# qiaozhijian/LPD-Net-Pytorch

Measured on NVIDIA B200. Metric: LPD-Net eval embedding throughput (featnet=lpdnet, 4096 pts, k=20, NetVLAD K=64 D=1024 -> 256), higher is better.
Workload: dtype f16

## Files before the change

### include/lpd_b200.h

```cpp
#ifndef LPD_B200_H
#define LPD_B200_H

#include <stddef.h>
#include <stdint.h>

#ifdef __cplusplus
extern "C" {
#endif

#define LPD_ABI_VERSION 2

typedef enum lpd_status {
    LPD_OK = 0,
    LPD_EINVAL = -1,
    LPD_EWORKSPACE = -2,
    LPD_ECUDA = -3,
    LPD_EUNSUPPORTED = -4
} lpd_status;

typedef enum lpd_act {
    LPD_ACT_NONE = 0,
    LPD_ACT_RELU = 1,
    LPD_ACT_LEAKY = 2,
    LPD_ACT_SIGMOID = 3,
// ... 3 lines not shown

#define LPD_A_MK 0
#define LPD_A_KM 1
#define LPD_B_NK 0
#define LPD_B_KN 1

int lpd_abi_version(void);
const char* lpd_status_str(int status);
const char* lpd_last_cuda_error(void);
int lpd_device_info(int* sm_count, int* cc_major, int* cc_minor, size_t* smem_optin_bytes);

int lpd_bn_fold(const float* gamma, const float* beta, const float* mean, const float* var,
                const float* bias, float eps, int C, float* scale, float* shift, void* stream);

int lpd_transpose(const float* in, float* out, int batch, int rows, int cols, void* stream);

int lpd_knn(const float* x, int B, int N, int C, int k, void* idx, int idx_i64, void* stream);

size_t lpd_knn_workspace_bytes(int B, int N, int C, int k);
int lpd_knn_tc(const float* x, int B, int N, int C, int k, void* idx, int idx_i64,
               void* workspace, size_t workspace_bytes, void* stream);
int lpd_knn_tc_variant(int v);
size_t lpd_knn_tc_flags_offset(int B, int N, int C, int k);

size_t lpd_knn_xyz_workspace_bytes(int B, int N);
int lpd_knn_xyz(const float* x, int B, int N, int k, void* idx, int idx_i64, void* workspace, size_t workspace_bytes,
                void* stream);

int lpd_cell_order(const float* x, int B, int N, int32_t* perm, int32_t* inv, float* xyz_sorted,
                   void* workspace, size_t workspace_bytes, void* stream);

int lpd_cell_order_grid(const float* x, int B, int N, int32_t* perm, int32_t* inv, float* xyz_sorted,
                        void* workspace, size_t workspace_bytes, void* stream);
int lpd_knn_xyz_ordered(int B, int N, int k, void* idx, int idx_i64, void* workspace, size_t workspace_bytes, void* stream);

int lpd_gemm(const float* A, int a_layout, int lda, long long strideA,
             const float* B, int b_layout, int ldb, long long strideB,
             float* C, int ldc, long long strideC,
             int M, int N, int K, int batch,
             const float* scale, const float* shift, int act, float slope, const float* aux,
             void* stream);

int lpd_gemm_tf32(const float* A, int lda, const float* B, int ldb, float* C, int ldc,
                  int M, int N, int K, const float* scale, const float* shift, int act, float slope,
                  void* stream);
int lpd_gemm_tf32_ex(const float* A, int lda, const float* B, int ldb, float* C, int ldc,
// ... 140 lines not shown
```

### lpd-net-pytorch_b200/_lib.py

```python
from __future__ import annotations

import ctypes as C
import os
from pathlib import Path

_HERE = Path(__file__).resolve().parent
LIB_PATH = _HERE / "liblpd_b200.so"

LPD_OK = 0
ACT_NONE, ACT_RELU, ACT_LEAKY, ACT_SIGMOID, ACT_GATE, ACT_ADD = 0, 1, 2, 3, 4, 5
A_MK, A_KM = 0, 1
B_NK, B_KN = 0, 1
ABI_VERSION = 2

_vp, _i, _f, _ll, _sz, _d = C.c_void_p, C.c_int, C.c_float, C.c_longlong, C.c_size_t, C.c_double

SIGNATURES = {
    "lpd_abi_version": (_i, []),
    "lpd_status_str": (C.c_char_p, [_i]),
    "lpd_last_cuda_error": (C.c_char_p, []),
    "lpd_device_info": (_i, [C.POINTER(_i), C.POINTER(_i), C.POINTER(_i), C.POINTER(_sz)]),
    "lpd_bn_fold": (_i, [_vp, _vp, _vp, _vp, _vp, _f, _i, _vp, _vp, _vp]),
    "lpd_transpose": (_i, [_vp, _vp, _i, _i, _i, _vp]),
    "lpd_knn": (_i, [_vp, _i, _i, _i, _i, _vp, _i, _vp]),
    "lpd_knn_workspace_bytes": (_sz, [_i, _i, _i, _i]),
    "lpd_knn_tc": (_i, [_vp, _i, _i, _i, _i, _vp, _i, _vp, _sz, _vp]),
    "lpd_knn_tc_variant": (_i, [_i]),
    "lpd_knn_tc_flags_offset": (_sz, [_i, _i, _i, _i]),
    "lpd_knn_xyz_workspace_bytes": (_sz, [_i, _i]),
    "lpd_knn_xyz": (_i, [_vp, _i, _i, _i, _vp, _i, _vp, _sz, _vp]),
    "lpd_cell_order": (_i, [_vp, _i, _i, _vp, _vp, _vp, _vp, _sz, _vp]),
    "lpd_cell_order_grid": (_i, [_vp, _i, _i, _vp, _vp, _vp, _vp, _sz, _vp]),
    "lpd_knn_xyz_ordered": (_i, [_i, _i, _i, _vp, _i, _vp, _sz, _vp]),
    "lpd_gemm": (_i, [_vp, _i, _i, _ll, _vp, _i, _i, _ll, _vp, _i, _ll, _i, _i, _i, _i,
                      _vp, _vp, _i, _f, _vp, _vp]),
    "lpd_gemm_tf32": (_i, [_vp, _i, _vp, _i, _vp, _i, _i, _i, _i, _vp, _vp, _i, _f, _vp]),
    "lpd_gemm_tf32_ex": (_i, [_vp, _i, _vp, _i, _vp, _i, _i, _i, _i, _i, _i, _vp, _vp, _i, _f, _vp]),
    "lpd_gemm_tf32_tn": (_i, [_vp, _i, _vp, _i, _vp, _i, _ll, _i, _i, _i, _i, _vp]),
    "lpd_gemm_f16": (_i, [_vp, _i, _vp, _i, _vp, _i, _i, _i, _i, _i, _vp, _vp, _i, _f, _vp]),
    "lpd_gemm_f16_tn": (_i, [_vp, _i, _vp, _i, _vp, _i, _ll, _i, _i, _i, _i, _vp]),
    "lpd_f32_to_f16": (_i, [_vp, _ll, _vp, _ll, _ll, _i, _vp]),
    "lpd_split3_tf32": (_i, [_vp, _ll, _vp, _i, _vp]),
    "lpd_transpose_split3": (_i, [_vp, _i, _ll, _i, _vp, _vp]),
    "lpd_gemm_tf32_out16": (_i, [_vp, _i, _vp, _i, _vp, _i, _i, _i, _i, _vp, _vp, _i, _f, _vp]),
    "lpd_softmax64_f16": (_i, [_vp, _ll, _vp, _vp]),
    "lpd_edge_gather_max_f16": (_i, [_vp, _i, _vp, _i, _vp, _i, _i, _i, _i, _i, _f, _vp, _i, _vp]),
    "lpd_edgeconv_dg20_f16": (_i, [_vp, _i, _vp, _i, _vp, _i, _i, _vp, _vp, _vp, _i, _f, _vp, _i, _vp, _i, _vp]),
    "lpd_edgeconv_dg32_f16": (_i, [_vp, _i, _vp, _i, _vp, _i, _i, _vp, _vp, _vp, _i, _f, _vp, _i, _vp, _i, _vp]),
    "lpd_pointwise_mlp2": (_i, [_vp, _i, _i, _ll, _vp, _vp, _vp, _vp, _vp, _vp, _i, _f, _vp, _i, _vp]),
    "lpd_colmax": (_i, [_vp, _i, _i, _i, _i, _vp, _vp]),
    "lpd_edge_gather_ext": (_i, [_vp, _i, _vp, _i, _vp, _i, _i, _i, _i, _vp, _vp, _i, _f, _vp, _i, _vp]),
# ... 82 lines not shown
```

### lpd-net-pytorch_b200/csrc/knn_tc.cu

```cuda
#include "tc_common.cuh"
#include "knn_select.cuh"

namespace lpd {

int knn_simt64_flagged(const float* x, int B, int N, int k, void* idx, int idx_i64, const int* flags, cudaStream_t st);

namespace tc {

constexpr int KT_Q = 128;
constexpr int KT_C = 64;
constexpr int KT_SCAN_WARPS = 8;
constexpr int KT_THREADS = 320;
constexpr int KT_STRIDE = 257;
constexpr int KT_BSTAGES = 3;
constexpr int KT_TSTAGES = 4;
constexpr int KT_XSLOTS = 8;

struct KnnTcParams {
    const float* xxpad;
    float* cand_v;
    int* cand_i;
    int B, N, Npad;
    int qtiles, ctiles;
};
// ... 335 lines not shown
struct KnnWs {
    size_t off_xx, off_r2, off_flags, off_x2, off_cv, off_ci, total;
    int npad, L;
    KnnWs(int B, int N, int k) {
        npad = (N + 127) / 128 * 128;
        L = k <= 24 ? 48 : 64;
        size_t o = 0;
        off_xx = o; o = align_up(o + (size_t)B * npad * 4, 256);
        off_r2 = o; o += (size_t)B * 4;
        off_flags = o; o = align_up(o + (size_t)B * ((N + 63) / 64) * 4, 256);
        off_x2 = o; o = align_up(o + (size_t)B * N * 128 * 4, 256);
        off_cv = o; o = align_up(o + (size_t)B * N * L * 4, 256);
        off_ci = o; o = align_up(o + (size_t)B * N * L * 4, 256);
        total = o;
    }
};

}
}

namespace lpd { namespace tc {
size_t knn2_workspace_bytes(int B, int N, int k);
size_t knn2_flags_offset(int B, int N, int k);
int knn2_run(const float* x, int B, int N, int k, void* idx, int idx_i64, void* workspace, size_t workspace_bytes, int mt,
             cudaStream_t st);
static int g_knn_variant = 1;
}}

extern "C" int lpd_knn_tc_variant(int v) {
    const int prev = lpd::tc::g_knn_variant;
    if (v >= 0 && v <= 3) lpd::tc::g_knn_variant = v;
    return prev;
}

extern "C" size_t lpd_knn_workspace_bytes(int B, int N, int C, int k) {
    if (B < 1 || N < 1 || C != 64 || k < 1 || k > 32) return 0;
    const size_t a = lpd::tc::KnnWs(B, N, k).total, b = lpd::tc::knn2_workspace_bytes(B, N, k);
    return a > b ? a : b;
}

extern "C" size_t lpd_knn_tc_flags_offset(int B, int N, int C, int k) {
    if (B < 1 || N < 1 || C != 64 || k < 1 || k > 32) return 0;
    return lpd::tc::g_knn_variant == 0 ? lpd::tc::KnnWs(B, N, k).off_flags : lpd::tc::knn2_flags_offset(B, N, k);
}

extern "C" int lpd_knn_tc(const float* x, int B, int N, int C, int k, void* idx, int idx_i64,
                          void* workspace, size_t workspace_bytes, void* stream) {
    using namespace lpd;
    LPD_REQUIRE(x && idx && workspace);
    LPD_REQUIRE(B >= 1 && B <= 65535 && N >= 1 && C == 64 && k >= 1 && k <= 32 && k <= N);
    LPD_REQUIRE((long long)B * N < (1ll << 31) / 128);
    LPD_REQUIRE(((uintptr_t)x & 15) == 0 && ((uintptr_t)workspace & 255) == 0);
    const tc::KnnWs W(B, N, k);
    if (workspace_bytes < lpd_knn_workspace_bytes(B, N, C, k)) return LPD_EWORKSPACE;
    int dev = 0, major = 0;
    LPD_CUDA_CHECK(cudaGetDevice(&dev));
    LPD_CUDA_CHECK(cudaDeviceGetAttribute(&major, cudaDevAttrComputeCapabilityMajor, dev));
    if (major != 10) return LPD_EUNSUPPORTED;
    cudaStream_t st = as_stream(stream);
    if (tc::g_knn_variant != 0) return tc::knn2_run(x, B, N, k, idx, idx_i64, workspace, workspace_bytes, tc::g_knn_variant, st);
    uint8_t* ws = reinterpret_cast<uint8_t*>(workspace);
    float* xxpad = reinterpret_cast<float*>(ws + W.off_xx);
    float* r2 = reinterpret_cast<float*>(ws + W.off_r2);
    int* flags = reinterpret_cast<int*>(ws + W.off_flags);
    float* x2 = reinterpret_cast<float*>(ws + W.off_x2);
    const int ftiles = (N + 63) / 64;
// ... 22 lines not shown
```

### lpd-net-pytorch_b200/csrc/knn_tc2.cu

```cuda
#include "tc_common.cuh"
#include <cuda_fp16.h>
#include <limits.h>
#include <stdlib.h>

namespace lpd {

int knn_simt64_list(const float* x, int B, int N, int k, void* idx, int idx_i64, const int* list, cudaStream_t st);

namespace tc {

constexpr int K2_C = 128;
constexpr int K2_BSTAGES = 4;
constexpr int K2_TCOLS = 512;
constexpr int K2_XSLOTS = 12;
constexpr int K2_TBL = 128;

struct Knn2Params {
    const float* nrmpad;
    const float* snpad;
    const uint4* xh;
    const uint4* ext;
    const float* xxpad;
    const float* r2;
    const float* r2c;
    const float* sc;
    int* cnt;
    int* cand;
    int B, N, Npad, k;
    int qtiles, ctiles;
};

__device__ __forceinline__ void tc_mma_f16(uint32_t tmem_d, uint64_t desc_a, uint64_t desc_b, uint32_t idesc, uint32_t accumulate) {
    asm volatile(
        "{\n\t.reg .pred p;\n\t"
        "setp.ne.b32 p, %4, 0;\n\t"
        "tcgen05.mma.cta_group::1.kind::f16 [%0], %1, %2, %3, p;\n\t}"
        ::"r"(tmem_d), "l"(desc_a), "l"(desc_b), "r"(idesc), "r"(accumulate)
        : "memory");
}
__device__ __forceinline__ void tc_mma_f16_p(uint32_t tmem_d, uint64_t desc_a, uint64_t desc_b, uint32_t idesc, uint32_t accumulate,
                                             uint32_t leader) {
    asm volatile(
        "{\n\t.reg .pred p, q;\n\t"
        "setp.ne.b32 p, %4, 0;\n\t"
        "elect.sync _|q, 0xffffffff;\n\t"
        "@q tcgen05.mma.cta_group::1.kind::f16 [%0], %1, %2, %3, p;\n\t}"
        ::"r"(tmem_d), "l"(desc_a), "l"(desc_b), "r"(idesc), "r"(accumulate), "r"(leader)
        : "memory");
}
__device__ __forceinline__ void tc_commit_p(uint64_t* bar, uint32_t leader) {
    asm volatile(
        "{\n\t.reg .pred q;\n\t"
// ... 262 lines not shown
    asm volatile(                                                                                                       \
        "tcgen05.ld.sync.aligned.32x32b.x32.b32 "                                                                       \
        "{%0, %1, %2, %3, %4, %5, %6, %7, %8, %9, %10, %11, %12, %13, %14, %15, "                                       \
        "%16, %17, %18, %19, %20, %21, %22, %23, %24, %25, %26, %27, %28, %29, %30, %31}, [%32];"                       \
        : "=r"(R[0]), "=r"(R[1]), "=r"(R[2]), "=r"(R[3]), "=r"(R[4]), "=r"(R[5]), "=r"(R[6]), "=r"(R[7]),              \
          "=r"(R[8]), "=r"(R[9]), "=r"(R[10]), "=r"(R[11]), "=r"(R[12]), "=r"(R[13]), "=r"(R[14]), "=r"(R[15]),        \
          "=r"(R[16]), "=r"(R[17]), "=r"(R[18]), "=r"(R[19]), "=r"(R[20]), "=r"(R[21]), "=r"(R[22]), "=r"(R[23]),      \
          "=r"(R[24]), "=r"(R[25]), "=r"(R[26]), "=r"(R[27]), "=r"(R[28]), "=r"(R[29]), "=r"(R[30]), "=r"(R[31])       \
        : "r"(ADDR))
    LPD_LD32(a, taddr);
    LPD_LD32(b, taddr + 64);
#undef LPD_LD32
    asm volatile("tcgen05.wait::ld.sync.aligned;" ::: "memory");
}
__device__ __forceinline__ int fkey(float v) {
    const int b = __float_as_int(v);
    return b ^ ((b >> 31) & 0x7fffffff);
}
__device__ __forceinline__ float fmax3(float a, float b, float c) {
    float r;
    asm("max.f32 %0, %1, %2, %3;" : "=f"(r) : "f"(a), "f"(b), "f"(c));
    return r;
}

template <int MT, bool TS = false>
struct K2Smem {
    static constexpr int SCAN_THREADS = 256 * MT;
    static constexpr int TSTAGES = TS ? 3 : K2_TCOLS / (K2_C * MT);
    static constexpr int EXS = SCAN_THREADS + 1;
    static constexpr uint32_t A_TILE = 128 * 128;
    static constexpr uint32_t A_BYTES = MT * A_TILE;
    static constexpr uint32_t B_BYTES = K2_C * 128;
    static constexpr uint32_t BX_BYTES = K2_C * 32;
    static constexpr size_t off_b = TS ? 0 : 2 * A_BYTES;
    static constexpr size_t off_bx = off_b + K2_BSTAGES * B_BYTES;
    static constexpr size_t off_ax = off_bx + K2_BSTAGES * BX_BYTES;
    static constexpr size_t off_xs = off_ax + 128 * 32;
    static constexpr size_t off_ex = off_xs + K2_XSLOTS * K2_C * 4;
    static constexpr size_t off_tbl = off_ex + (size_t)32 * EXS * 4;
    static constexpr size_t off_bar = (off_tbl + (size_t)8 * MT * K2_TBL * 4 + 7) / 8 * 8;
    static constexpr size_t total = off_bar + (4 + 2 * K2_BSTAGES + 2 * TSTAGES) * 8 + 16;
    static_assert(total <= 227 * 1024, "knn2 shared memory budget");
};

template <int MT, int CAP, bool TIGHT, bool TS>
__global__ void __launch_bounds__(256 * MT + 64, 1)
knn2_tc_kernel(const __grid_constant__ CUtensorMap tmap_a, const __grid_constant__ CUtensorMap tmap_b, Knn2Params P) {
    static_assert(!TS || MT == 1, "TS mode: one 128-row query tile per item");
    using S = K2Smem<MT, TS>;
    constexpr int SCAN_WARPS = 8 * MT;
    constexpr uint32_t ACOL = 384;
    constexpr int TCOLS = K2_C * MT;
    constexpr int K2_TSTAGES = S::TSTAGES;
    extern __shared__ __align__(1024) uint8_t smem[];
    if ((smem_u32(smem) & 1023u) != 0) __trap();
    uint8_t* a_s = smem;
    uint8_t* b_s = smem + S::off_b;
    uint8_t* bx_s = smem + S::off_bx;
    uint8_t* ax_s = smem + S::off_ax;
    float* xs = reinterpret_cast<float*>(smem + S::off_xs);
    float* ex = reinterpret_cast<float*>(smem + S::off_ex);
    int* tbl = reinterpret_cast<int*>(smem + S::off_tbl);
    uint64_t* afull = reinterpret_cast<uint64_t*>(smem + S::off_bar);
    uint64_t* aempty = afull + 2;
    uint64_t* bfull = aempty + 2;
    uint64_t* bempty = bfull + K2_BSTAGES;
    uint64_t* tfull = bempty + K2_BSTAGES;
    uint64_t* tempty = tfull + K2_TSTAGES;
    uint32_t* tmem_slot = reinterpret_cast<uint32_t*>(tempty + K2_TSTAGES);

    const int warp = threadIdx.x >> 5, lane = threadIdx.x & 31;
    const int items = P.B * P.qtiles;
    const int nstages = 2 * P.ctiles;
    const int full_blocks = P.N >> 6;

    if (threadIdx.x < 128) {
        const int r = threadIdx.x;
        const __half2 h01 = __floats2half2_rn(64.f, 0.03125f), h23 = __floats2half2_rn(6.103515625e-05f, 32768.f);
        uint4* e = reinterpret_cast<uint4*>(ax_s) + (r >> 3) * 16 + (r & 7);
        e[0] = make_uint4(*reinterpret_cast<const uint32_t*>(&h01), *reinterpret_cast<const uint32_t*>(&h23), 0u, 0u);
        e[8] = make_uint4(0u, 0u, 0u, 0u);
        asm volatile("fence.proxy.async.shared::cta;" ::: "memory");
    }
    if (warp == SCAN_WARPS + 1) {
        if (lane == 0) {
            asm volatile("prefetch.tensormap [%0];" ::"l"(reinterpret_cast<uint64_t>(&tmap_a)) : "memory");
            asm volatile("prefetch.tensormap [%0];" ::"l"(reinterpret_cast<uint64_t>(&tmap_b)) : "memory");
            for (int s = 0; s < 2; ++s) { mbar_init(&afull[s], TS ? SCAN_WARPS : 1); mbar_init(&aempty[s], 1); }
            for (int s = 0; s < K2_BSTAGES; ++s) { mbar_init(&bfull[s], 1); mbar_init(&bempty[s], 1); }
            for (int s = 0; s < K2_TSTAGES; ++s) { mbar_init(&tfull[s], 1); mbar_init(&tempty[s], SCAN_WARPS); }
            asm volatile("fence.mbarrier_init.release.cluster;" ::: "memory");
        }
        __syncwarp();
        asm volatile("tcgen05.alloc.cta_group::1.sync.aligned.shared::cta.b32 [%0], %1;" ::"r"(smem_u32(tmem_slot)), "r"(TS ? 512 : TCOLS * K2_TSTAGES) : "memory");
        asm volatile("tcgen05.relinquish_alloc_permit.cta_group::1.sync.aligned;" ::: "memory");
    }
    tc_fence_before();
    __syncthreads();
    tc_fence_after();
    const uint32_t tmem_base = *tmem_slot;

    if (warp == SCAN_WARPS) {
        {
            const uint32_t leader = lane == 0;
            uint32_t tcount = 0, icount = 0;
            for (int item = blockIdx.x; item < items; item += gridDim.x, ++icount) {
                const int b = item / P.qtiles, q0 = (item % P.qtiles) * (128 * MT);
                const uint32_t ab = icount & 1, aph = (icount >> 1) & 1;
                if (!TS) {
                    mbar_wait_sleep(&aempty[ab], aph ^ 1);
                    mbar_expect_tx_p(&afull[ab], S::A_BYTES, leader);
#pragma unroll
                    for (int mt = 0; mt < MT; ++mt)
                        tma_load_2d_p(a_s + ab * S::A_BYTES + mt * S::A_TILE, &tmap_a, &afull[ab], 0, b * P.N + q0 + mt * 128, leader);
                }
                const uint4* extb = P.ext + (size_t)b * (P.Npad >> 6) * 128;
                const float* snb = P.snpad + (size_t)b * P.Npad;
                uint32_t s = tcount % K2_BSTAGES, ph = (tcount / K2_BSTAGES) & 1, xsl = tcount % K2_XSLOTS;
                for (int cs = 0; cs < nstages; ++cs, ++tcount) {
                    const int ct = cs >= P.ctiles ? cs - P.ctiles : cs;
                    mbar_wait_sleep(&bempty[s], ph ^ 1);
                    mbar_expect_tx_p(&bfull[s], S::B_BYTES + S::BX_BYTES + (TIGHT ? K2_C * 4 : 0), leader);
                    tma_load_2d_p(b_s + s * S::B_BYTES, &tmap_b, &bfull[s], 0, b * P.N + ct * K2_C, leader);
                    bulk_load_p(bx_s + s * S::BX_BYTES, extb + (size_t)ct * 256, S::BX_BYTES, &bfull[s], leader);
                    if (TIGHT) bulk_load_p(xs + xsl * K2_C, snb + ct * K2_C, K2_C * 4, &bfull[s], leader);
                    if (++s == K2_BSTAGES) { s = 0; ph ^= 1; }
                    xsl = (xsl + 1) % K2_XSLOTS;
                }
            }
        }
    } else if (warp == SCAN_WARPS + 1) {
        {
            constexpr uint32_t idesc = make_idesc_f16(128, K2_C);
            const uint32_t leader = lane == 0;
            const uint64_t dax = make_smem_desc_ext(smem_u32(ax_s));
            uint32_t tcount = 0, icount = 0;
            for (int item = blockIdx.x; item < items; item += gridDim.x, ++icount) {
                const uint32_t ab = icount & 1, aph = (icount >> 1) & 1;
                mbar_wait_sleep(&afull[ab], aph);
                if (TS) tc_fence_after();
                const uint64_t da0 = make_smem_desc(smem_u32(a_s + ab * S::A_BYTES));
                const uint32_t ta0 = tmem_base + ACOL + ab * 64;
                uint32_t s = tcount % K2_BSTAGES, ph = (tcount / K2_BSTAGES) & 1;
                uint32_t ts = tcount % K2_TSTAGES, tph = (tcount / K2_TSTAGES) & 1;
                for (int cs = 0; cs < nstages; ++cs, ++tcount) {
                    mbar_wait(&tempty[ts], tph ^ 1);
                    mbar_wait(&bfull[s], ph);
                    tc_fence_after();
                    const uint64_t db = make_smem_desc(smem_u32(b_s + s * S::B_BYTES));
                    const uint64_t dbx = make_smem_desc_ext(smem_u32(bx_s + s * S::BX_BYTES));
                    if (TS) {
                        const uint32_t d = tmem_base + ts * TCOLS;
#pragma unroll
                        for (int ks = 0; ks < 4; ++ks) tc_mma_f16_ts(d, ta0 + ks * 8, db + (uint64_t)(ks * 2), idesc, ks ? 1u : 0u);
                        tc_mma_f16_ts(d, ta0 + 32, dbx, idesc, 1u);
                    } else {
#pragma unroll
                        for (int ks = 0; ks < 5; ++ks) {
#pragma unroll
                            for (int mt = 0; mt < MT; ++mt) {
                                const uint64_t da = da0 + (uint64_t)(mt * (S::A_TILE >> 4));
                                const uint32_t d = tmem_base + ts * TCOLS + mt * K2_C;
                                if (ks < 4) tc_mma_f16_p(d, da + (uint64_t)(ks * 2), db + (uint64_t)(ks * 2), idesc, ks ? 1u : 0u, leader);
                                else tc_mma_f16_p(d, dax, dbx, idesc, 1u, leader);
                            }
                        }
                    }
                    tc_commit_p(&bempty[s], leader);
                    tc_commit_p(&tfull[ts], leader);
                    if (++s == K2_BSTAGES) { s = 0; ph ^= 1; }
                    if (++ts == K2_TSTAGES) { ts = 0; tph ^= 1; }
                }
                tc_commit_p(&aempty[ab], leader);
            }
        }
    } else {
        const int quad = warp & 3, half = (warp >> 2) & 1, mt = warp >> 3;
        const int own = mt * 256 + half * 128 + quad * 32 + lane;
        const int partner = own ^ 128;
        const uint32_t tm_lane = ((uint32_t)(quad * 32) << 16) + mt * K2_C + half * 32;
        uint32_t tcount = 0, icount = 0;
        uint4 aw[5];
        auto load_a = [&](int it2) {
            const int b2 = it2 / P.qtiles, q02 = (it2 % P.qtiles) * 128;
            const long long grow = (long long)b2 * P.N + q02 + quad * 32 + lane;
            const bool inb = grow < (long long)P.B * P.N;
            const uint4* src = P.xh + grow * 8;
            const uint4 zero = make_uint4(0u, 0u, 0u, 0u);
            if (half == 0) {
#pragma unroll
                for (int i = 0; i < 5; ++i) aw[i] = inb ? __ldg(src + i) : zero;
            } else {
#pragma unroll
                for (int i = 0; i < 3; ++i) aw[i] = inb ? __ldg(src + 5 + i) : zero;
                const __half2 h01 = __floats2half2_rn(64.f, 0.03125f), h23 = __floats2half2_rn(6.103515625e-05f, 32768.f);
// ... 71 lines not shown
                }
            }
            bitonic_sort32_desc(m);
#pragma unroll
            for (int j = 0; j < 32; ++j) ex[j * S::EXS + own] = m[j];
            named_bar(1, S::SCAN_THREADS);
#pragma unroll
            for (int j = 0; j < 32; ++j) m[j] = fmaxf(m[j], ex[(31 - j) * S::EXS + partner]);
            named_bar(2, S::SCAN_THREADS);
            bitonic_merge32_desc(m);
            float tau0 = m[0];
#pragma unroll
            for (int j = 1; j < 32; ++j) tau0 = (j == P.k - 1) ? m[j] : tau0;
            float thr = INFINITY;
            if (live) {
                const float xxi = __ldg(P.xxpad + (size_t)b * P.Npad + row);
                const float r2 = __ldg(P.r2 + b), r2c = __ldg(P.r2c + b), sigma = __ldg(P.sc + 2 * b);
                const float rc = sqrtf(r2c);
                float eps = (1.9e-6f / sigma) * (ni + rc) + 7.62939453125e-6f * (xxi + r2) + 3.814697265625e-6f * r2c;
                if (!TIGHT) eps += 2.5e-3f * ni * rc;
                thr = fmaxf(tau0 - 2.f * eps * inv_cb, -1.0e9f);
                if (!(eps * inv_cb < INFINITY)) thr = __int_as_float(0x7fc00000);
            }
            if (have_next) store_a(icount + 1);
            const int dthr = __reduce_max_sync(kFull, fkey(live ? gself - thr : -INFINITY));
            int cnt = 0;
            int* mine = P.cand + (((size_t)b * P.N + (live ? row : 0)) * 2 + half) * CAP;
            for (int cs = 0; cs < P.ctiles; ++cs, ++tcount) {
                const uint32_t ts = tcount % K2_TSTAGES, tph = (tcount / K2_TSTAGES) & 1;
                mbar_wait(&tfull[ts], tph);
                if (use_tbl && wtbl[cs] > dthr) {
                    __syncwarp();
                    if (lane == 0) mbar_arrive(&tempty[ts]);
                    continue;
                }
                tc_fence_after();
                uint32_t r0[32], r1[32];
                tc_ld32x2(tmem_base + tm_lane + ts * TCOLS, r0, r1);
                tc_fence_before();
                __syncwarp();
                if (lane == 0) mbar_arrive(&tempty[ts]);
                float u0[32], u1[32];
                if (TIGHT) {
                    const float* xsj = xs + (tcount % K2_XSLOTS) * K2_C + half * 32;
#pragma unroll
                    for (int j = 0; j < 32; j += 4) {
                        const float4 s0 = *reinterpret_cast<const float4*>(xsj + j), s1 = *reinterpret_cast<const float4*>(xsj + 64 + j);
                        u0[j + 0] = fmaf(cni, s0.x, __uint_as_float(r0[j + 0])); u1[j + 0] = fmaf(cni, s1.x, __uint_as_float(r1[j + 0]));
                        u0[j + 1] = fmaf(cni, s0.y, __uint_as_float(r0[j + 1])); u1[j + 1] = fmaf(cni, s1.y, __uint_as_float(r1[j + 1]));
                        u0[j + 2] = fmaf(cni, s0.z, __uint_as_float(r0[j + 2])); u1[j + 2] = fmaf(cni, s1.z, __uint_as_float(r1[j + 2]));
                        u0[j + 3] = fmaf(cni, s0.w, __uint_as_float(r0[j + 3])); u1[j + 3] = fmaf(cni, s1.w, __uint_as_float(r1[j + 3]));
// ... 330 lines not shown
    LPD_LAUNCH_CHECK();
    return LPD_OK;
}

static int make_tmap_f16(CUtensorMap* m, const __half* base, long long rows, int box_rows) {
    EncodeTiledFn enc = get_encode();
    if (!enc) { snprintf(g_last_error, sizeof(g_last_error), "cuTensorMapEncodeTiled entry point not found"); return LPD_ECUDA; }
    cuuint64_t dims[2] = {64u, (cuuint64_t)rows};
    cuuint64_t strides[1] = {128u};
    cuuint32_t box[2] = {64u, (cuuint32_t)box_rows};
    cuuint32_t estr[2] = {1, 1};
    CUresult r = enc(m, CU_TENSOR_MAP_DATA_TYPE_FLOAT16, 2, const_cast<__half*>(base), dims, strides, box, estr,
                     CU_TENSOR_MAP_INTERLEAVE_NONE, CU_TENSOR_MAP_SWIZZLE_128B, CU_TENSOR_MAP_L2_PROMOTION_L2_256B,
                     CU_TENSOR_MAP_FLOAT_OOB_FILL_NONE);
    if (r != CUDA_SUCCESS) { snprintf(g_last_error, sizeof(g_last_error), "cuTensorMapEncodeTiled (fp16) failed: CUresult %d", (int)r); return LPD_ECUDA; }
    return LPD_OK;
}

static inline size_t align_up2(size_t v, size_t a) { return (v + a - 1) / a * a; }

static int g_cap_small = [] { const char* e = getenv("LPD_KNN_CAP"); return (e && atoi(e) == 40) ? 40 : 64; }();

struct Knn2Ws {
    size_t off_xx, off_nrm, off_sn, off_ext, off_r2, off_r2c, off_mu, off_sc, off_flags, off_list, off_xh, off_cnt, off_cand, total;
    int npad, cap;
    Knn2Ws(int B, int N, int k) {
        npad = (N + 255) / 256 * 256;
        cap = k > 24 ? 128 : (g_cap_small == 40 ? 40 : 64);
        size_t o = 0;
        off_xx = o; o = align_up2(o + (size_t)B * npad * 4, 256);
        off_nrm = o; o = align_up2(o + (size_t)B * npad * 4, 256);
        off_sn = o; o = align_up2(o + (size_t)B * npad * 4, 256);
        off_ext = o; o = align_up2(o + (size_t)B * npad * 32, 256);
        off_r2 = o; o += (size_t)B * 4;
        off_r2c = o; o = align_up2(o + (size_t)B * 4, 256);
        off_mu = o; o = align_up2(o + (size_t)B * K2_CSPLIT * 196 * 4, 256);
        off_sc = o; o = align_up2(o + (size_t)B * 2 * 4, 256);
        off_flags = o; o = align_up2(o + (size_t)B * ((N + 63) / 64) * 4, 256);
        off_list = o; o = align_up2(o + ((size_t)B * ((N + 63) / 64) + 1) * 4, 256);
        off_xh = o; o = align_up2(o + (size_t)B * N * 64 * 2, 256);
        off_cnt = o; o = align_up2(o + (size_t)B * N * 2 * 4, 256);
        off_cand = o; o = align_up2(o + (size_t)B * N * 2 * cap * 4, 256);
        total = o;
    }
};

size_t knn2_workspace_bytes(int B, int N, int k) { return Knn2Ws(B, N, k).total; }

template <int MT, int CAP, bool TIGHT, bool TS = false>
static int knn2_launch(const CUtensorMap& ta, const CUtensorMap& tb, const Knn2Params& P, cudaStream_t st) {
    const size_t smem = K2Smem<MT, TS>::total;
    LPD_CUDA_CHECK(allow_smem(knn2_tc_kernel<MT, CAP, TIGHT, TS>, smem));
    int dev = 0, sms = 0;
    LPD_CUDA_CHECK(cudaGetDevice(&dev));
    LPD_CUDA_CHECK(cudaDeviceGetAttribute(&sms, cudaDevAttrMultiProcessorCount, dev));
    const int items = P.B * P.qtiles;
    knn2_tc_kernel<MT, CAP, TIGHT, TS><<<items < sms ? items : sms, 256 * MT + 64, smem, st>>>(ta, tb, P);
    LPD_LAUNCH_CHECK();
    return LPD_OK;
}

int knn2_run(const float* x, int B, int N, int k, void* idx, int idx_i64, void* workspace, size_t workspace_bytes, int mt,
             cudaStream_t st) {
    const Knn2Ws W(B, N, k);
    if (workspace_bytes < W.total) return LPD_EWORKSPACE;
    uint8_t* ws = reinterpret_cast<uint8_t*>(workspace);
    float* xxpad = reinterpret_cast<float*>(ws + W.off_xx);
    float* nrmpad = reinterpret_cast<float*>(ws + W.off_nrm);
    float* snpad = reinterpret_cast<float*>(ws + W.off_sn);
    float* r2 = reinterpret_cast<float*>(ws + W.off_r2);
    float* r2c = reinterpret_cast<float*>(ws + W.off_r2c);
    float* mu = reinterpret_cast<float*>(ws + W.off_mu);
    float* sc = reinterpret_cast<float*>(ws + W.off_sc);
    int* flags = reinterpret_cast<int*>(ws + W.off_flags);
    int* list = reinterpret_cast<int*>(ws + W.off_list);
    __half* xh = reinterpret_cast<__half*>(ws + W.off_xh);
    LPD_CUDA_CHECK(cudaMemsetAsync(r2, 0, W.off_mu - W.off_r2, st));
    LPD_CUDA_CHECK(cudaMemsetAsync(flags, 0, W.off_list - W.off_flags + sizeof(int), st));
    knn2_center_kernel<<<dim3(K2_CSPLIT, B), 256, 0, st>>>(x, N, mu);
    LPD_LAUNCH_CHECK();
    static bool prep_smem_ok = false;
    if (!prep_smem_ok) { LPD_CUDA_CHECK(allow_smem(knn2_prep_kernel, K2_PREP_SMEM)); prep_smem_ok = true; }
    knn2_prep_kernel<<<dim3(ceil_div(W.npad, 256), B), 256, K2_PREP_SMEM, st>>>(x, mu, sc, N, W.npad, xh, reinterpret_cast<uint4*>(ws + W.off_ext), xxpad, nrmpad, snpad, r2, r2c);
    LPD_LAUNCH_CHECK();
    CUtensorMap ta, tb;
    int rc = make_tmap_f16(&ta, xh, (long long)B * N, 128);
    if (rc != LPD_OK) return rc;
    rc = make_tmap_f16(&tb, xh, (long long)B * N, K2_C);
    if (rc != LPD_OK) return rc;
    Knn2Params P;
    P.nrmpad = nrmpad; P.snpad = snpad; P.ext = reinterpret_cast<const uint4*>(ws + W.off_ext); P.xh = reinterpret_cast<const uint4*>(xh); P.xxpad = xxpad; P.r2 = r2; P.r2c = r2c; P.sc = sc;
    P.cnt = reinterpret_cast<int*>(ws + W.off_cnt);
    P.cand = reinterpret_cast<int*>(ws + W.off_cand);
    P.B = B; P.N = N; P.Npad = W.npad; P.k = k;
    P.qtiles = ceil_div(N, mt == 2 ? 256 : 128); P.ctiles = ceil_div(N, K2_C);
    if (mt == 3) {
        rc = (W.cap == 40) ? knn2_launch<1, 40, false, true>(ta, tb, P, st)
                           : (k <= 24 ? knn2_launch<1, 64, false, true>(ta, tb, P, st) : knn2_launch<1, 128, true, true>(ta, tb, P, st));
    } else if (W.cap == 40) rc = (mt == 2) ? knn2_launch<2, 40, false>(ta, tb, P, st) : knn2_launch<1, 40, false>(ta, tb, P, st);
    else if (k <= 24) rc = (mt == 2) ? knn2_launch<2, 64, false>(ta, tb, P, st) : knn2_launch<1, 64, false>(ta, tb, P, st);
    else             rc = (mt == 2) ? knn2_launch<2, 128, true>(ta, tb, P, st) : knn2_launch<1, 128, true>(ta, tb, P, st);
    if (rc != LPD_OK) return rc;
    rc = (W.cap == 40) ? knn2_refine_launch<40>(x, xxpad, P.cnt, P.cand, B, N, W.npad, k, idx, idx_i64, flags, list, st)
         : (W.cap == 64 ? knn2_refine_launch<64>(x, xxpad, P.cnt, P.cand, B, N, W.npad, k, idx, idx_i64, flags, list, st)
                        : knn2_refine_launch<128>(x, xxpad, P.cnt, P.cand, B, N, W.npad, k, idx, idx_i64, flags, list, st));
    if (rc != LPD_OK) return rc;
    return knn_simt64_list(x, B, N, k, idx, idx_i64, list, st);
}

size_t knn2_flags_offset(int B, int N, int k) { return Knn2Ws(B, N, k).off_flags; }
size_t knn2_cnt_offset(int B, int N, int k) { return Knn2Ws(B, N, k).off_cnt; }

}
}
```

### lpd-net-pytorch_b200/ops.py

```python
from __future__ import annotations

import torch

from . import _lib
from ._lib import (ACT_ADD, ACT_GATE, ACT_LEAKY, ACT_NONE, ACT_RELU, ACT_SIGMOID, A_KM, A_MK, B_KN, B_NK)

__all__ = ["bn_fold", "transpose", "knn", "knn_tc_variant", "pointwise_mlp2", "gemm", "colmax", "edge_gather_ext", "edgeconv_dg",
           "gemm_tf32", "linear", "set_precision", "get_precision", "netvlad_assign", "softmax64", "netvlad_finish", "splitk_reduce", "quadruplet_loss", "retrieval_topk", "retrieval_tc", "retrieval_search", "recall_count",
           "ACT_NONE", "ACT_RELU", "ACT_LEAKY", "ACT_SIGMOID", "ACT_GATE", "A_MK", "A_KM", "B_NK", "B_KN"]


def _stream() -> int:
    return torch.cuda.current_stream().cuda_stream


_weights_epoch = 0


def weights_epoch() -> int:
    return _weights_epoch


def bump_weights_epoch() -> None:
    global _weights_epoch
    _weights_epoch += 1


def dispatch_key() -> tuple:
    return (_precision, SPATIAL_ORDER, KNN_TENSOR_CORES, KNN_GRID, knn_tc_variant(-1) if _lib._lib is not None else -1)

# ... 53 lines not shown
    out = torch.empty(2, C, device=mean.device, dtype=torch.float32)
    _call("lpd_bn_fold", 1, lib.lpd_bn_fold, _p(gamma), _p(beta), _p(mean), _p(var), _p(bias), float(eps), C,
                               out[0].data_ptr(), out[1].data_ptr(), _stream())
    return out[0], out[1]


def transpose(x: torch.Tensor) -> torch.Tensor:
    lib = _lib.load()
    x = _f32(x, "x").contiguous()
    b, R, Cc = x.shape
    out = torch.empty(b, Cc, R, device=x.device, dtype=torch.float32)
    _call("lpd_transpose", 1, lib.lpd_transpose, x.data_ptr(), out.data_ptr(), b, R, Cc, _stream())
    return out


KNN_TENSOR_CORES = True
KNN_GRID = True


def knn_tc_variant(v: int = -1) -> int:
    return int(_lib.load().lpd_knn_tc_variant(int(v)))


def knn(x_pm: torch.Tensor, k: int, int64: bool = False, diag: dict | None = None) -> torch.Tensor:
    lib = _lib.load()
    x_pm = _f32(x_pm, "x").contiguous()
    B, N, Cc = x_pm.shape
    idx = torch.empty(B, N, k, device=x_pm.device, dtype=torch.int64 if int64 else torch.int32)
    if KNN_TENSOR_CORES and Cc == 64 and N >= 128 and x_pm.data_ptr() % 16 == 0:
        nbytes = lib.lpd_knn_workspace_bytes(B, N, Cc, k)
        ws = torch.empty((nbytes + 3) // 4, device=x_pm.device, dtype=torch.float32)
        _call(f"lpd_knn_tc[C={Cc},k={k}]", 5, lib.lpd_knn_tc, x_pm.data_ptr(), B, N, Cc, k, idx.data_ptr(), int(int64),
              ws.data_ptr(), ws.numel() * 4, _stream())
        if diag is not None:
            off = lib.lpd_knn_tc_flags_offset(B, N, Cc, k) // 4
            diag["flagged_tiles"] = int((ws.view(torch.int32)[off: off + B * ((N + 63) // 64)] != 0).sum().item())
            diag["tiles"] = B * ((N + 63) // 64)
    elif KNN_GRID and Cc == 3 and N >= 64 and _grid_of(x_pm) is not None:
        ws = _grid_of(x_pm)
        _call(f"lpd_knn_xyz[k={k}]", 2, lib.lpd_knn_xyz_ordered, B, N, k, idx.data_ptr(), int(int64), ws.data_ptr(), ws.numel() * 4, _stream())
    elif KNN_GRID and Cc == 3 and N >= 64:
        nbytes = lib.lpd_knn_xyz_workspace_bytes(B, N)
        ws = torch.empty((nbytes + 3) // 4, device=x_pm.device, dtype=torch.float32)
        _call(f"lpd_knn_xyz[k={k}]", 2, lib.lpd_knn_xyz, x_pm.data_ptr(), B, N, k, idx.data_ptr(), int(int64), ws.data_ptr(),
              ws.numel() * 4, _stream())
    else:
        _call(f"lpd_knn[C={Cc},k={k}]", 1, lib.lpd_knn, x_pm.data_ptr(), B, N, Cc, k, idx.data_ptr(), int(int64), _stream())
    return idx


SPATIAL_ORDER = True


_grid_cache = None


def _grid_of(x_pm: torch.Tensor):
    c = _grid_cache
    if (c is not None and x_pm.data_ptr() == c[0].data_ptr() and tuple(x_pm.shape) == tuple(c[0].shape) and c[0]._version == c[2]
            and x_pm.device == c[0].device):
# ... 594 lines not shown
```

Measured before the change: 29330.

## Skip pass-two kNN candidate tiles via shared stage bitmask across producer warps

The tensor-core kNN kernel's second pass previously reloaded and recomputed every candidate tile. Scan warps now build a 128-bit mask of tiles whose lower bound is within the threshold and pass it through new mbarriers. The TMA loader and MMA warps then only load and multiply the listed tiles. This cuts pass-two TMA traffic and MMA work, at the cost of an extra ballot/reduction plus barrier handoff and a longer pipeline critical path. It also adds an optional stage counter for diagnostics.

```diff
diff --git a/include/lpd_b200.h b/include/lpd_b200.h
--- a/include/lpd_b200.h
+++ b/include/lpd_b200.h
@@ -49,6 +49,10 @@
                void* workspace, size_t workspace_bytes, void* stream);
 int lpd_knn_tc_variant(int v);
 size_t lpd_knn_tc_flags_offset(int B, int N, int C, int k);
+int lpd_knn_tc_stage_list(int v);
+int lpd_knn_tc_count_stages(int v);
+size_t lpd_knn_tc_cnt_offset(int B, int N, int C, int k);
+size_t lpd_knn_tc_stage_count_offset(int B, int N, int C, int k);
 
 size_t lpd_knn_xyz_workspace_bytes(int B, int N);
 int lpd_knn_xyz(const float* x, int B, int N, int k, void* idx, int idx_i64, void* workspace, size_t workspace_bytes,
diff --git a/lpd-net-pytorch_b200/_lib.py b/lpd-net-pytorch_b200/_lib.py
--- a/lpd-net-pytorch_b200/_lib.py
+++ b/lpd-net-pytorch_b200/_lib.py
@@ -27,6 +27,10 @@
     "lpd_knn_tc": (_i, [_vp, _i, _i, _i, _i, _vp, _i, _vp, _sz, _vp]),
     "lpd_knn_tc_variant": (_i, [_i]),
     "lpd_knn_tc_flags_offset": (_sz, [_i, _i, _i, _i]),
+    "lpd_knn_tc_stage_list": (_i, [_i]),
+    "lpd_knn_tc_count_stages": (_i, [_i]),
+    "lpd_knn_tc_cnt_offset": (_sz, [_i, _i, _i, _i]),
+    "lpd_knn_tc_stage_count_offset": (_sz, [_i, _i, _i, _i]),
     "lpd_knn_xyz_workspace_bytes": (_sz, [_i, _i]),
     "lpd_knn_xyz": (_i, [_vp, _i, _i, _i, _vp, _i, _vp, _sz, _vp]),
     "lpd_cell_order": (_i, [_vp, _i, _i, _vp, _vp, _vp, _vp, _sz, _vp]),
diff --git a/lpd-net-pytorch_b200/csrc/knn_tc.cu b/lpd-net-pytorch_b200/csrc/knn_tc.cu
--- a/lpd-net-pytorch_b200/csrc/knn_tc.cu
+++ b/lpd-net-pytorch_b200/csrc/knn_tc.cu
@@ -381,6 +381,10 @@
 namespace lpd { namespace tc {
 size_t knn2_workspace_bytes(int B, int N, int k);
 size_t knn2_flags_offset(int B, int N, int k);
+size_t knn2_cnt_offset(int B, int N, int k);
+size_t knn2_nstage2_offset(int B, int N, int k);
+int knn2_stage_list(int v);
+int knn2_count_stages(int v);
 int knn2_run(const float* x, int B, int N, int k, void* idx, int idx_i64, void* workspace, size_t workspace_bytes, int mt,
              cudaStream_t st);
 static int g_knn_variant = 1;
@@ -401,6 +405,19 @@
 extern "C" size_t lpd_knn_tc_flags_offset(int B, int N, int C, int k) {
     if (B < 1 || N < 1 || C != 64 || k < 1 || k > 32) return 0;
     return lpd::tc::g_knn_variant == 0 ? lpd::tc::KnnWs(B, N, k).off_flags : lpd::tc::knn2_flags_offset(B, N, k);
+}
+
+extern "C" int lpd_knn_tc_stage_list(int v) { return lpd::tc::knn2_stage_list(v); }
+extern "C" int lpd_knn_tc_count_stages(int v) { return lpd::tc::knn2_count_stages(v); }
+
+extern "C" size_t lpd_knn_tc_cnt_offset(int B, int N, int C, int k) {
+    if (B < 1 || N < 1 || C != 64 || k < 1 || k > 32) return 0;
+    return lpd::tc::knn2_cnt_offset(B, N, k);
+}
+
+extern "C" size_t lpd_knn_tc_stage_count_offset(int B, int N, int C, int k) {
+    if (B < 1 || N < 1 || C != 64 || k < 1 || k > 32) return 0;
+    return lpd::tc::knn2_nstage2_offset(B, N, k);
 }
 
 extern "C" int lpd_knn_tc(const float* x, int B, int N, int C, int k, void* idx, int idx_i64,
diff --git a/lpd-net-pytorch_b200/csrc/knn_tc2.cu b/lpd-net-pytorch_b200/csrc/knn_tc2.cu
--- a/lpd-net-pytorch_b200/csrc/knn_tc2.cu
+++ b/lpd-net-pytorch_b200/csrc/knn_tc2.cu
@@ -26,8 +26,10 @@
     const float* sc;
     int* cnt;
     int* cand;
+    unsigned long long* nstage2;
     int B, N, Npad, k;
     int qtiles, ctiles;
+    int list;
 };
 
 __device__ __forceinline__ void tc_mma_f16(uint32_t tmem_d, uint64_t desc_a, uint64_t desc_b, uint32_t idesc, uint32_t accumulate) {
@@ -336,6 +338,15 @@
     asm("max.f32 %0, %1, %2, %3;" : "=f"(r) : "f"(a), "f"(b), "f"(c));
     return r;
 }
+__device__ __forceinline__ int k2_next_stage(const uint4& lm, int cs) {
+    const uint32_t w[4] = {lm.x, lm.y, lm.z, lm.w};
+#pragma unroll
+    for (int i = 0; i < 4; ++i) {
+        const uint32_t v = (cs >> 5) > i ? 0u : ((cs >> 5) < i ? w[i] : w[i] & (0xffffffffu << (cs & 31)));
+        if (v) return 32 * i + __ffs(v) - 1;
+    }
+    return INT_MAX;
+}
 
 template <int MT, bool TS = false>
 struct K2Smem {
@@ -352,8 +363,10 @@
     static constexpr size_t off_xs = off_ax + 128 * 32;
     static constexpr size_t off_ex = off_xs + K2_XSLOTS * K2_C * 4;
     static constexpr size_t off_tbl = off_ex + (size_t)32 * EXS * 4;
-    static constexpr size_t off_bar = (off_tbl + (size_t)8 * MT * K2_TBL * 4 + 7) / 8 * 8;
-    static constexpr size_t total = off_bar + (4 + 2 * K2_BSTAGES + 2 * TSTAGES) * 8 + 16;
+    static constexpr size_t off_wm = off_tbl + (size_t)8 * MT * K2_TBL * 4;
+    static constexpr size_t off_lm = off_wm + (size_t)8 * MT * K2_TBL / 8;
+    static constexpr size_t off_bar = (off_lm + (size_t)2 * K2_TBL / 8 + 7) / 8 * 8;
+    static constexpr size_t total = off_bar + (8 + 2 * K2_BSTAGES + 2 * TSTAGES) * 8 + 16;
     static_assert(total <= 227 * 1024, "knn2 shared memory budget");
 };
 
@@ -375,9 +388,13 @@
     float* xs = reinterpret_cast<float*>(smem + S::off_xs);
     float* ex = reinterpret_cast<float*>(smem + S::off_ex);
     int* tbl = reinterpret_cast<int*>(smem + S::off_tbl);
+    uint4* wm = reinterpret_cast<uint4*>(smem + S::off_wm);
+    uint4* lm = reinterpret_cast<uint4*>(smem + S::off_lm);
     uint64_t* afull = reinterpret_cast<uint64_t*>(smem + S::off_bar);
     uint64_t* aempty = afull + 2;
-    uint64_t* bfull = aempty + 2;
+    uint64_t* lfull = aempty + 2;
+    uint64_t* lempty = lfull + 2;
+    uint64_t* bfull = lempty + 2;
     uint64_t* bempty = bfull + K2_BSTAGES;
     uint64_t* tfull = bempty + K2_BSTAGES;
     uint64_t* tempty = tfull + K2_TSTAGES;
@@ -385,8 +402,9 @@
 
     const int warp = threadIdx.x >> 5, lane = threadIdx.x & 31;
     const int items = P.B * P.qtiles;
-    const int nstages = 2 * P.ctiles;
     const int full_blocks = P.N >> 6;
+    static_assert(K2_TBL == 128, "the stage list is one uint4 of bits");
+    const bool listed = P.list && P.ctiles <= K2_TBL;
 
     if (threadIdx.x < 128) {
         const int r = threadIdx.x;
@@ -400,7 +418,10 @@
         if (lane == 0) {
             asm volatile("prefetch.tensormap [%0];" ::"l"(reinterpret_cast<uint64_t>(&tmap_a)) : "memory");
             asm volatile("prefetch.tensormap [%0];" ::"l"(reinterpret_cast<uint64_t>(&tmap_b)) : "memory");
-            for (int s = 0; s < 2; ++s) { mbar_init(&afull[s], TS ? SCAN_WARPS : 1); mbar_init(&aempty[s], 1); }
+            for (int s = 0; s < 2; ++s) {
+                mbar_init(&afull[s], TS ? SCAN_WARPS : 1); mbar_init(&aempty[s], 1);
+                mbar_init(&lfull[s], 1); mbar_init(&lempty[s], 2);
+            }
             for (int s = 0; s < K2_BSTAGES; ++s) { mbar_init(&bfull[s], 1); mbar_init(&bempty[s], 1); }
             for (int s = 0; s < K2_TSTAGES; ++s) { mbar_init(&tfull[s], 1); mbar_init(&tempty[s], SCAN_WARPS); }
             asm volatile("fence.mbarrier_init.release.cluster;" ::: "memory");
@@ -413,6 +434,13 @@
     __syncthreads();
     tc_fence_after();
     const uint32_t tmem_base = *tmem_slot;
+    auto take_list = [&](uint32_t ab, uint32_t aph) -> uint4 {
+        mbar_wait(&lfull[ab], aph);
+        const uint4 l = lm[ab];
+        __syncwarp();
+        if (lane == 0) mbar_arrive(&lempty[ab]);
+        return l;
+    };
 
     if (warp == SCAN_WARPS) {
         {
@@ -430,17 +458,21 @@
                 }
                 const uint4* extb = P.ext + (size_t)b * (P.Npad >> 6) * 128;
                 const float* snb = P.snpad + (size_t)b * P.Npad;
-                uint32_t s = tcount % K2_BSTAGES, ph = (tcount / K2_BSTAGES) & 1, xsl = tcount % K2_XSLOTS;
-                for (int cs = 0; cs < nstages; ++cs, ++tcount) {
-                    const int ct = cs >= P.ctiles ? cs - P.ctiles : cs;
+                auto load_stage = [&](int ct) {
+                    const uint32_t s = tcount % K2_BSTAGES, ph = (tcount / K2_BSTAGES) & 1, xsl = tcount % K2_XSLOTS;
                     mbar_wait_sleep(&bempty[s], ph ^ 1);
                     mbar_expect_tx_p(&bfull[s], S::B_BYTES + S::BX_BYTES + (TIGHT ? K2_C * 4 : 0), leader);
                     tma_load_2d_p(b_s + s * S::B_BYTES, &tmap_b, &bfull[s], 0, b * P.N + ct * K2_C, leader);
                     bulk_load_p(bx_s + s * S::BX_BYTES, extb + (size_t)ct * 256, S::BX_BYTES, &bfull[s], leader);
                     if (TIGHT) bulk_load_p(xs + xsl * K2_C, snb + ct * K2_C, K2_C * 4, &bfull[s], leader);
-                    if (++s == K2_BSTAGES) { s = 0; ph ^= 1; }
-                    xsl = (xsl + 1) % K2_XSLOTS;
-                }
+                    ++tcount;
+                };
+                for (int ct = 0; ct < P.ctiles; ++ct) load_stage(ct);
+                const uint4 l = listed ? take_list(ab, aph) : make_uint4(0u, 0u, 0u, 0u);
+                int n2 = 0;
+                for (int ct = listed ? k2_next_stage(l, 0) : 0; ct < P.ctiles; ct = listed ? k2_next_stage(l, ct + 1) : ct + 1, ++n2)
+                    load_stage(ct);
+                if (P.nstage2 && lane == 0 && n2) atomicAdd(P.nstage2, (unsigned long long)n2);
             }
         }
     } else if (warp == SCAN_WARPS + 1) {
@@ -455,9 +487,9 @@
                 if (TS) tc_fence_after();
                 const uint64_t da0 = make_smem_desc(smem_u32(a_s + ab * S::A_BYTES));
                 const uint32_t ta0 = tmem_base + ACOL + ab * 64;
-                uint32_t s = tcount % K2_BSTAGES, ph = (tcount / K2_BSTAGES) & 1;
-                uint32_t ts = tcount % K2_TSTAGES, tph = (tcount / K2_TSTAGES) & 1;
-                for (int cs = 0; cs < nstages; ++cs, ++tcount) {
+                auto mma_stage = [&]() {
+                    const uint32_t s = tcount % K2_BSTAGES, ph = (tcount / K2_BSTAGES) & 1;
+                    const uint32_t ts = tcount % K2_TSTAGES, tph = (tcount / K2_TSTAGES) & 1;
                     mbar_wait(&tempty[ts], tph ^ 1);
                     mbar_wait(&bfull[s], ph);
                     tc_fence_after();
@@ -482,9 +514,15 @@
                     }
                     tc_commit_p(&bempty[s], leader);
                     tc_commit_p(&tfull[ts], leader);
-                    if (++s == K2_BSTAGES) { s = 0; ph ^= 1; }
-                    if (++ts == K2_TSTAGES) { ts = 0; tph ^= 1; }
-                }
+                    ++tcount;
+                };
+                for (int cs = 0; cs < P.ctiles; ++cs) mma_stage();
+                int n2 = P.ctiles;
+                if (listed) {
+                    const uint4 l = take_list(ab, aph);
+                    n2 = __popc(l.x) + __popc(l.y) + __popc(l.z) + __popc(l.w);
+                }
+                for (int i = 0; i < n2; ++i) mma_stage();
                 tc_commit_p(&aempty[ab], leader);
             }
         }
@@ -602,11 +640,36 @@
                 thr = fmaxf(tau0 - 2.f * eps * inv_cb, -1.0e9f);
                 if (!(eps * inv_cb < INFINITY)) thr = __int_as_float(0x7fc00000);
             }
+            const int dthr = __reduce_max_sync(kFull, fkey(live && !isnan(thr) ? gself - thr : -INFINITY));
+            uint4 l = make_uint4(0u, 0u, 0u, 0u);
+            if (listed) {
+                uint32_t w[4];
+#pragma unroll
+                for (int i = 0; i < 4; ++i) {
+                    const int cs = 32 * i + lane;
+                    w[i] = __ballot_sync(kFull, cs < P.ctiles && wtbl[cs] <= dthr);
+                }
+                if (lane == 0) wm[warp] = make_uint4(w[0], w[1], w[2], w[3]);
+                named_bar(3, S::SCAN_THREADS);
+#pragma unroll 4
+                for (int v = 0; v < SCAN_WARPS; ++v) {
+                    const uint4 t = wm[v];
+                    l.x |= t.x; l.y |= t.y; l.z |= t.z; l.w |= t.w;
+                }
+                if (warp == 0) {
+                    const uint32_t ab = icount & 1;
+                    mbar_wait(&lempty[ab], ((icount >> 1) & 1) ^ 1);
+                    if (lane == 0) {
+                        lm[ab] = l;
+                        mbar_arrive(&lfull[ab]);
+                    }
+                    __syncwarp();
+                }
+            }
             if (have_next) store_a(icount + 1);
-            const int dthr = __reduce_max_sync(kFull, fkey(live ? gself - thr : -INFINITY));
             int cnt = 0;
             int* mine = P.cand + (((size_t)b * P.N + (live ? row : 0)) * 2 + half) * CAP;
-            for (int cs = 0; cs < P.ctiles; ++cs, ++tcount) {
+            for (int cs = listed ? k2_next_stage(l, 0) : 0; cs < P.ctiles; cs = listed ? k2_next_stage(l, cs + 1) : cs + 1, ++tcount) {
                 const uint32_t ts = tcount % K2_TSTAGES, tph = (tcount / K2_TSTAGES) & 1;
                 mbar_wait(&tfull[ts], tph);
                 if (use_tbl && wtbl[cs] > dthr) {
@@ -983,7 +1046,7 @@
 static int g_cap_small = [] { const char* e = getenv("LPD_KNN_CAP"); return (e && atoi(e) == 40) ? 40 : 64; }();
 
 struct Knn2Ws {
-    size_t off_xx, off_nrm, off_sn, off_ext, off_r2, off_r2c, off_mu, off_sc, off_flags, off_list, off_xh, off_cnt, off_cand, total;
+    size_t off_xx, off_nrm, off_sn, off_ext, off_r2, off_r2c, off_mu, off_sc, off_flags, off_list, off_n2, off_xh, off_cnt, off_cand, total;
     int npad, cap;
     Knn2Ws(int B, int N, int k) {
         npad = (N + 255) / 256 * 256;
@@ -999,6 +1062,7 @@
         off_sc = o; o = align_up2(o + (size_t)B * 2 * 4, 256);
         off_flags = o; o = align_up2(o + (size_t)B * ((N + 63) / 64) * 4, 256);
         off_list = o; o = align_up2(o + ((size_t)B * ((N + 63) / 64) + 1) * 4, 256);
+        off_n2 = o; o = align_up2(o + 8, 256);
         off_xh = o; o = align_up2(o + (size_t)B * N * 64 * 2, 256);
         off_cnt = o; o = align_up2(o + (size_t)B * N * 2 * 4, 256);
         off_cand = o; o = align_up2(o + (size_t)B * N * 2 * cap * 4, 256);
@@ -1007,6 +1071,9 @@
 };
 
 size_t knn2_workspace_bytes(int B, int N, int k) { return Knn2Ws(B, N, k).total; }
+
+static int g_stage_list = 1;
+static int g_count_stages = 0;
 
 template <int MT, int CAP, bool TIGHT, bool TS = false>
 static int knn2_launch(const CUtensorMap& ta, const CUtensorMap& tb, const Knn2Params& P, cudaStream_t st) {
@@ -1053,6 +1120,12 @@
     P.nrmpad = nrmpad; P.snpad = snpad; P.ext = reinterpret_cast<const uint4*>(ws + W.off_ext); P.xh = reinterpret_cast<const uint4*>(xh); P.xxpad = xxpad; P.r2 = r2; P.r2c = r2c; P.sc = sc;
     P.cnt = reinterpret_cast<int*>(ws + W.off_cnt);
     P.cand = reinterpret_cast<int*>(ws + W.off_cand);
+    P.nstage2 = nullptr;
+    if (g_count_stages) {
+        P.nstage2 = reinterpret_cast<unsigned long long*>(ws + W.off_n2);
+        LPD_CUDA_CHECK(cudaMemsetAsync(P.nstage2, 0, sizeof(unsigned long long), st));
+    }
+    P.list = g_stage_list;
     P.B = B; P.N = N; P.Npad = W.npad; P.k = k;
     P.qtiles = ceil_div(N, mt == 2 ? 256 : 128); P.ctiles = ceil_div(N, K2_C);
     if (mt == 3) {
@@ -1071,6 +1144,17 @@
 
 size_t knn2_flags_offset(int B, int N, int k) { return Knn2Ws(B, N, k).off_flags; }
 size_t knn2_cnt_offset(int B, int N, int k) { return Knn2Ws(B, N, k).off_cnt; }
-
-}
-}
+size_t knn2_nstage2_offset(int B, int N, int k) { return Knn2Ws(B, N, k).off_n2; }
+int knn2_stage_list(int v) {
+    const int prev = g_stage_list;
+    if (v == 0 || v == 1) g_stage_list = v;
+    return prev;
+}
+int knn2_count_stages(int v) {
+    const int prev = g_count_stages;
+    if (v == 0 || v == 1) g_count_stages = v;
+    return prev;
+}
+
+}
+}
diff --git a/lpd-net-pytorch_b200/ops.py b/lpd-net-pytorch_b200/ops.py
--- a/lpd-net-pytorch_b200/ops.py
+++ b/lpd-net-pytorch_b200/ops.py
@@ -5,7 +5,7 @@
 from . import _lib
 from ._lib import (ACT_ADD, ACT_GATE, ACT_LEAKY, ACT_NONE, ACT_RELU, ACT_SIGMOID, A_KM, A_MK, B_KN, B_NK)
 
-__all__ = ["bn_fold", "transpose", "knn", "knn_tc_variant", "pointwise_mlp2", "gemm", "colmax", "edge_gather_ext", "edgeconv_dg",
+__all__ = ["bn_fold", "transpose", "knn", "knn_tc_variant", "knn_tc_stage_list", "knn_tc_count_stages","pointwise_mlp2", "gemm", "colmax", "edge_gather_ext", "edgeconv_dg",
            "gemm_tf32", "linear", "set_precision", "get_precision", "netvlad_assign", "softmax64", "netvlad_finish", "splitk_reduce", "quadruplet_loss", "retrieval_topk", "retrieval_tc", "retrieval_search", "recall_count",
            "ACT_NONE", "ACT_RELU", "ACT_LEAKY", "ACT_SIGMOID", "ACT_GATE", "A_MK", "A_KM", "B_NK", "B_KN"]
 
@@ -105,6 +105,14 @@
     return int(_lib.load().lpd_knn_tc_variant(int(v)))
 
 
+def knn_tc_stage_list(v: int = -1) -> int:
+    return int(_lib.load().lpd_knn_tc_stage_list(int(v)))
+
+
+def knn_tc_count_stages(v: int = -1) -> int:
+    return int(_lib.load().lpd_knn_tc_count_stages(int(v)))
+
+
 def knn(x_pm: torch.Tensor, k: int, int64: bool = False, diag: dict | None = None) -> torch.Tensor:
     lib = _lib.load()
     x_pm = _f32(x_pm, "x").contiguous()
@@ -119,6 +127,15 @@
             off = lib.lpd_knn_tc_flags_offset(B, N, Cc, k) // 4
             diag["flagged_tiles"] = int((ws.view(torch.int32)[off: off + B * ((N + 63) // 64)] != 0).sum().item())
             diag["tiles"] = B * ((N + 63) // 64)
+            variant = knn_tc_variant(-1)
+            if variant != 0:
+                off = lib.lpd_knn_tc_cnt_offset(B, N, Cc, k) // 4
+                diag["cnt"] = ws.view(torch.int32)[off: off + B * N * 2].view(B, N, 2).cpu().numpy()
+                if lib.lpd_knn_tc_count_stages(-1):
+                    off = lib.lpd_knn_tc_stage_count_offset(B, N, Cc, k) // 4
+                    diag["pass2_stages"] = int(ws.view(torch.int32)[off: off + 2].view(torch.int64).item())
+                    rows = 256 if variant == 2 else 128
+                    diag["pass2_stages_all"] = B * ((N + rows - 1) // rows) * ((N + 127) // 128)
     elif KNN_GRID and Cc == 3 and N >= 64 and _grid_of(x_pm) is not None:
         ws = _grid_of(x_pm)
         _call(f"lpd_knn_xyz[k={k}]", 2, lib.lpd_knn_xyz_ordered, B, N, k, idx.data_ptr(), int(int64), ws.data_ptr(), ws.numel() * 4, _stream())
```

Result: faster. 29870, median of 6 (+1.8%).
